# christianhbye/21cmVAE

Hardware: AMD Instinct MI355X
Metric: emulated signals/sec (batched predict) (higher is better)
Workload: dtype f16 (f32 accumulate)

## Files before the change

### 21cmvae_amd/_native.py

```python
import ctypes as C
import os
import threading
import weakref

import numpy as np

HERE = os.path.dirname(os.path.abspath(__file__))
LIB_PATH = os.environ.get("V21_LIB") or os.path.join(HERE, "libv21.so")

PREC_F32, PREC_F16, PREC_BF16 = 0, 1, 2
PRECISIONS = {"f32": PREC_F32, "fp32": PREC_F32, "float32": PREC_F32,
              "f16": PREC_F16, "fp16": PREC_F16, "float16": PREC_F16,
              "bf16": PREC_BF16, "bfloat16": PREC_BF16}
ACT_LINEAR, ACT_RELU, ACT_GAUSS = 0, 1, 2
FWD_IN_TRANSFORM, FWD_OUT_TRANSFORM, FWD_FORCE_GENERIC, FWD_NO_SMALL, FWD_FORCE_CHAIN, FWD_FORCE_JIT = 1, 2, 4, 8, 16, 32
COMM_ID_BYTES = 128


class EngineUnavailable(RuntimeError):
    """libv21.so cannot be loaded or no MI355X is visible."""


class EngineError(RuntimeError):
    """A v21_* call returned a negative status."""
# ... 40 lines not shown


class SampleOut(C.Structure):
    _fields_ = [(k, C.c_void_p) for k in SAMPLE_OUTPUTS]


_P = C.c_void_p
_F = C.POINTER(C.c_float)
SIGNATURES = {
    "v21_last_error": (C.c_char_p, []),
    "v21_version": (C.c_int, []),
    "v21_device_count": (C.c_int, [C.POINTER(C.c_int)]),
    "v21_ctx_create": (C.c_int, [C.c_int, C.POINTER(_P)]),
    "v21_ctx_destroy": (C.c_int, [_P]),
    "v21_ctx_sync": (C.c_int, [_P]),
    "v21_ctx_set_stream": (C.c_int, [_P, _P]),
    "v21_ctx_get_stream": (C.c_int, [_P, C.POINTER(_P)]),
    "v21_malloc": (C.c_int, [_P, C.c_size_t, C.POINTER(_P)]),
    "v21_free": (C.c_int, [_P, _P]),
    "v21_memcpy_h2d": (C.c_int, [_P, _P, _P, C.c_size_t]),
    "v21_memcpy_d2h": (C.c_int, [_P, _P, _P, C.c_size_t]),
    "v21_memset": (C.c_int, [_P, _P, C.c_int, C.c_size_t]),
    "v21_event_create": (C.c_int, [_P, C.POINTER(_P)]),
    "v21_event_destroy": (C.c_int, [_P, _P]),
    "v21_event_record": (C.c_int, [_P, _P]),
    "v21_event_elapsed_ms": (C.c_int, [_P, _P, _P, C.POINTER(C.c_float)]),
    "v21_mlp_create": (C.c_int, [_P, C.c_int, C.POINTER(C.c_int), C.POINTER(C.c_int), C.POINTER(_P)]),
    "v21_mlp_destroy": (C.c_int, [_P]),
    "v21_mlp_num_params": (C.c_int, [_P, C.POINTER(C.c_size_t)]),
    "v21_mlp_set_weights": (C.c_int, [_P, _F, C.c_size_t]),
    "v21_mlp_get_weights": (C.c_int, [_P, _F, C.c_size_t]),
    "v21_mlp_set_input_transform": (C.c_int, [_P, C.POINTER(AffineIn)]),
    "v21_mlp_set_output_transform": (C.c_int, [_P, C.POINTER(AffineOut)]),
    "v21_mlp_has_fused": (C.c_int, [_P, C.c_int, C.POINTER(C.c_int)]),
    "v21_mlp_jit": (C.c_int, [_P, C.c_int, C.c_int, C.POINTER(C.c_int)]),
    "v21_jit_prebuild": (C.c_int, [C.c_int, C.POINTER(C.c_int), C.POINTER(C.c_int), C.c_int, C.c_char_p]),
    "v21_mlp_forward": (C.c_int, [_P, _P, C.c_int, C.c_int64, _F, C.c_int, C.c_int]),
    "v21_mlp_forward_dev": (C.c_int, [_P, _P, C.c_int64, C.c_int64, _P, C.c_int64, C.c_int, C.c_int]),
    "v21_trainer_create": (C.c_int, [_P, C.c_int, C.c_int, C.POINTER(_P)]),
    "v21_trainer_destroy": (C.c_int, [_P]),
    "v21_trainer_set_adam": (C.c_int, [_P, C.POINTER(Adam)]),
    "v21_trainer_set_lr": (C.c_int, [_P, C.c_float]),
    "v21_trainer_get_lr": (C.c_int, [_P, C.POINTER(C.c_float)]),
    "v21_trainer_set_data": (C.c_int, [_P, C.c_int, _F, _F, _F, C.c_int64]),
    "v21_trainer_run_epoch": (C.c_int, [_P, C.POINTER(C.c_int32), C.c_int, C.POINTER(C.c_double)]),
    "v21_trainer_eval": (C.c_int, [_P, C.c_int, C.c_int, C.POINTER(C.c_double)]),
    "v21_trainer_step_dev": (C.c_int, [_P, _P, _P, _P, C.c_int, C.c_int]),
    "v21_trainer_last_step_loss": (C.c_int, [_P, C.POINTER(C.c_double)]),
    "v21_trainer_get_state": (C.c_int, [_P, C.POINTER(C.c_int64), _F, _F, C.c_size_t]),
    "v21_trainer_set_state": (C.c_int, [_P, C.c_int64, _F, _F, C.c_size_t]),
    "v21_trainer_get_grad": (C.c_int, [_P, _F, C.c_size_t]),
    "v21_trainer_use_graph": (C.c_int, [_P, C.c_int]),
    "v21_debug_poison_lds": (C.c_int, [_P, C.c_uint32]),
    "v21_debug_check_chain_jobs": (C.c_int, [_P, C.c_longlong, C.c_longlong]),
    "v21_debug_trainer_counters": (C.c_int, [_P, C.POINTER(C.c_longlong)]),
    "v21_route_forward": (C.c_int, [C.c_int, C.POINTER(C.c_int), C.POINTER(C.c_int), C.c_int, C.c_int64, C.c_int, C.c_int, C.POINTER(C.c_int)]),
    "v21_route_train": (C.c_int, [C.c_int, C.POINTER(C.c_int), C.POINTER(C.c_int), C.c_int, C.c_int, C.c_int, C.c_int, C.c_int,
                                  C.POINTER(C.c_int), C.POINTER(C.c_int)]),
    "v21_trainer_jit": (C.c_int, [_P, C.c_int, C.POINTER(C.c_int)]),
    "v21_mlp_last_route": (C.c_int, [_P, C.POINTER(C.c_int), C.POINTER(C.c_longlong)]),
    "v21_mlp_jacobian": (C.c_int, [_P, _P, C.c_int, C.c_int64, _F, _F, C.c_int, C.c_int]),
    "v21_mlp_jacobian_dev": (C.c_int, [_P, _P, C.c_int64, C.c_int64, _P, C.c_int64, _P, C.c_int, C.c_int]),
    "v21_mlp_set_likelihood": (C.c_int, [_P, _F, _F, C.c_int32]),
    "v21_mlp_loglike": (C.c_int, [_P, _P, C.c_int, C.c_int64, _F, _F, C.c_int, C.c_int]),
    "v21_mlp_loglike_dev": (C.c_int, [_P, _P, C.c_int64, C.c_int64, _P, _P, C.c_int, C.c_int]),
    "v21_route_jacobian": (C.c_int, [C.c_int, C.POINTER(C.c_int), C.POINTER(C.c_int), C.c_int, C.c_int64, C.c_int, C.POINTER(C.c_int)]),
    "v21_mlp_last_jac_route": (C.c_int, [_P, C.POINTER(C.c_int), C.POINTER(C.c_longlong)]),
    "v21_mlp_fisher": (C.c_int, [_P, _P, C.c_int, C.c_int64, _F, _F, _F, C.c_int, C.c_int]),
    "v21_mlp_fisher_dev": (C.c_int, [_P, _P, C.c_int64, C.c_int64, _P, _P, _P, C.c_int, C.c_int]),
    "v21_mlp_fit": (C.c_int, [_P, _P, C.c_int, C.c_int64, _F, C.c_int64, C.POINTER(FitOpts), _P, _F, _F, _F, C.POINTER(C.c_int32),
                              C.c_int, C.c_int]),
    "v21_mlp_fit_dev": (C.c_int, [_P, _P, C.c_int64, C.c_int64, _P, C.c_int64, C.POINTER(FitOpts), _P, _P, _P, _P, _P, C.c_int, C.c_int]),
    "v21_mlp_sample": (C.c_int, [_P, _P, C.c_int, C.c_int64, _F, C.c_int64, C.POINTER(SampleOpts), _P, C.POINTER(SampleOut),
                                 C.c_int, C.c_int]),
    "v21_mlp_sample_dev": (C.c_int, [_P, _P, C.c_int64, C.c_int64, _P, C.c_int64, C.POINTER(SampleOpts), _P, C.POINTER(SampleOut),
                                     C.c_int, C.c_int]),
    "v21_nuisance_whiten": (C.c_int, [C.POINTER(C.c_double), _F, C.c_int32, C.c_int32, C.POINTER(C.c_double), C.POINTER(C.c_double)]),
    "v21_mlp_set_nuisance": (C.c_int, [_P, C.POINTER(C.c_double), C.c_int32, C.c_int32]),
    "v21_mlp_nuisance_info": (C.c_int, [_P, C.POINTER(C.c_int32)]),
    "v21_mlp_nuisance_coef": (C.c_int, [_P, _P, C.c_int, C.c_int64, C.POINTER(C.c_double), C.c_int, C.c_int]),
    "v21_trainer_last_route": (C.c_int, [_P, C.POINTER(C.c_int), C.POINTER(C.c_int), C.POINTER(C.c_longlong), C.POINTER(C.c_longlong)]),
    "v21_route_name": (C.c_char_p, [C.c_int, C.c_int]),
    "v21_trainer_get_data_dev": (C.c_int, [_P, C.c_int, C.POINTER(_P), C.POINTER(_P), C.POINTER(_P), C.POINTER(C.c_int64)]),
    "v21_debug_clock_probe_start": (C.c_int, [_P, C.c_double, C.c_double]),
    "v21_debug_forward_clocked": (C.c_int, [_P, _P, C.c_int64, C.c_int64, _P, C.c_int64, C.c_int, C.c_int, _P]),
    "v21_debug_clock_probe_read": (C.c_int, [_P, C.POINTER(C.c_double), C.POINTER(C.c_double), C.POINTER(C.c_double), C.POINTER(C.c_int)]),
    "v21_trainer_set_vae": (C.c_int, [_P, C.c_float, C.c_int, C.c_uint64]),
    "v21_trainer_enable_stamps": (C.c_int, [_P, C.c_int]),
    "v21_trainer_chain_stamps": (C.c_int, [_P, C.POINTER(C.c_uint64), C.c_int]),
    "v21_host_alloc": (C.c_int, [_P, C.c_size_t, C.POINTER(_P)]),
    "v21_host_free": (C.c_int, [_P, _P]),
    "v21_sweep_create": (C.c_int, [C.POINTER(_P), C.c_int, C.POINTER(_P)]),
    "v21_sweep_destroy": (C.c_int, [_P]),
    "v21_sweep_run_epoch": (C.c_int, [_P, C.POINTER(C.c_int32), C.c_int, C.POINTER(C.c_double)]),
    "v21_joint_create": (C.c_int, [_P, _P, C.c_int, C.POINTER(_P)]),
    "v21_joint_destroy": (C.c_int, [_P]),
    "v21_joint_run_epoch": (C.c_int, [_P, C.POINTER(C.c_int32), C.c_int, C.POINTER(C.c_double)]),
    "v21_joint_eval": (C.c_int, [_P, C.POINTER(C.c_double)]),
    "v21_comm_get_unique_id": (C.c_int, [_P, _P]),
    "v21_comm_init": (C.c_int, [_P, C.c_int, C.c_int, _P]),
    "v21_comm_init_host": (C.c_int, [_P, C.c_int, C.c_int, C.POINTER(CommHostOps)]),
    "v21_comm_destroy": (C.c_int, [_P]),
    "v21_comm_init_null": (C.c_int, [_P, C.c_int, C.c_int]),
    "v21_comm_set_buckets": (C.c_int, [_P, C.c_int]),
    "v21_trainer_phase_timing": (C.c_int, [_P, C.c_int, C.c_int]),
    "v21_trainer_phase_times": (C.c_int, [_P, C.POINTER(C.c_double), C.POINTER(C.c_int)]),
# ... 824 lines not shown
```

### 21cmvae_amd/csrc/api_forward.hip

```cpp
#include "api_internal.h"

namespace v21 {
#define V21_DECL(a)                                                      \
  hipError_t launch_fused_##a##_F32(const FusedArgs&, hipStream_t);      \
  hipError_t launch_fused_##a##_F16x2sp(const FusedArgs&, hipStream_t);  \
  hipError_t launch_fused_##a##_BF16x2sp(const FusedArgs&, hipStream_t);
V21_ARCH_LIST(V21_DECL)
#undef V21_DECL
hipError_t launch_fused_S1_F16x2spClk(const FusedArgs&, hipStream_t);
hipError_t launch_fused_S1_BF16x2spClk(const FusedArgs&, hipStream_t);
}

typedef hipError_t (*fused_launcher)(const FusedArgs&, hipStream_t);
struct FusedEntry {
  int L;
  const int* dims;
  const int* act;
  fused_launcher fn[3];
};
#define V21_ENTRY(a) \
  {Arch##a::L, Arch##a::dims, Arch##a::act, {launch_fused_##a##_F32, launch_fused_##a##_F16x2sp, launch_fused_##a##_BF16x2sp}},
static const FusedEntry g_fused[] = {V21_ARCH_LIST(V21_ENTRY)};
#undef V21_ENTRY

// ... 329 lines not shown
  hipError_t rt = hipSuccess;
  if (route == FWD_FUSED || route == FWD_FUSED_RT) {
    CHK(ensure_stream(m, precision));
    a.x = d_x; a.ldx = ldx; a.y = d_y; a.ldy = ldy; a.n_rows = n;
    a.stream = m->d_stream[precision];
    const bool tout = (flags & V21_FWD_OUT_TRANSFORM) != 0;
    a.out_std = tout ? m->out_std : 1.0f;
    a.out_mean_scale = tout ? 1.0f : 0.0f;
    a.in_transform = (flags & V21_FWD_IN_TRANSFORM) ? 1 : 0;
    if (a.in_transform) a.tin = m->tin;
#ifdef V21_FUSED_STAMP
    a.dbg = (unsigned long long*)(getenv("V21_FUSED_DBG_PTR") ? strtoull(getenv("V21_FUSED_DBG_PTR"), nullptr, 0) : 0ull);
#endif
  }
  if (route == FWD_FUSED_RT) {
    rt = v21::jit_launch(jk, m->ctx->device, a, m->ctx->stream);
    if (rt != hipSuccess) (void)hipGetLastError();
    if (rt != hipSuccess && !force_jit) { q.jit = 0; route = decide_forward(q); }
  }
  note_route(m, route);
  if (route == FWD_TABLE) return forward_chain(m, d_x, ldx, n, d_y, ldy, precision, flags);
  if (route == FWD_GENERIC) return forward_generic(m, d_x, ldx, n, d_y, ldy, precision, flags);
  if (route == FWD_FUSED_RT) {
    if (rt == hipSuccess) return V21_OK;
    std::string why;
    v21::jit_state(jk, &why);
    return fail(V21_ERR_UNSUPPORTED, "V21_FWD_FORCE_JIT: %s (%s)", why.c_str(), hipGetErrorString(rt));
  }
  if (m->clk_stamps) {
    a.dbg = m->clk_stamps;
    HIPCHK((precision == V21_PREC_F16 ? launch_fused_S1_F16x2spClk : launch_fused_S1_BF16x2spClk)(a, m->ctx->stream));
    return V21_OK;
  }
  HIPCHK(g_fused[m->fused_id].fn[precision](a, m->ctx->stream));
  return V21_OK;
}
extern "C" int v21_mlp_forward_dev(v21_mlp* m, const float* d_x, int64_t ldx, int64_t n, float* d_y, int64_t ldy,
                                   int precision, int flags) {
  CHK(fwd_args(m, d_x && d_y, true, n, ldx, ldy, V21_DTYPE_F32, precision, flags));
  return n == 0 ? V21_OK : forward_rows(m, d_x, ldx, n, d_y, ldy, precision, flags);
}
extern "C" int v21_debug_forward_clocked(v21_mlp* m, const float* d_x, int64_t ldx, int64_t n, float* d_y, int64_t ldy, int precision,
                                         int flags, unsigned long long* d_stamps) {
  if (!m || !d_stamps) return fail(V21_ERR_ARG, "null argument");
  if (m->fused_id < 0 || g_fused[m->fused_id].dims != ArchS1::dims || (precision != V21_PREC_F16 && precision != V21_PREC_BF16))
    return fail(V21_ERR_UNSUPPORTED, "clock-stamped kernels exist for the headline stack (archs.h S1) in f16 / bf16 only");
  if (flags & (V21_FWD_FORCE_GENERIC | V21_FWD_FORCE_CHAIN | V21_FWD_FORCE_JIT)) return fail(V21_ERR_ARG, "route flags do not apply");
  m->clk_stamps = d_stamps;
  const int r = v21_mlp_forward_dev(m, d_x, ldx, n, d_y, ldy, precision, flags | V21_FWD_NO_SMALL);
  m->clk_stamps = nullptr;
  return r;
}

extern "C" int v21_mlp_jit(v21_mlp* m, int precision, int wait_ms, int* status) {
  if (!m || !status) return fail(V21_ERR_ARG, "null argument");
  if (precision < 0 || precision > 2) return fail(V21_ERR_ARG, "precision %d unknown", precision);
  *status = -1;
  if (m->fused_id >= 0) { *status = 1; return V21_OK; }
  std::string why;
  if (!v21::jit_eligible(m->L, m->dims.data(), m->act.data(), &why)) return fail(V21_ERR_UNSUPPORTED, "no fused kernel for this stack: %s", why.c_str());
  v21::JitKernel* k = jit_kernel(m, precision);
  if (!k) return fail(V21_ERR_UNSUPPORTED, "run-time compilation is switched off (V21_JIT=0) and no cached kernel exists");
  int s = v21::jit_state(k);
  if (s == v21::JIT_COMPILING && wait_ms != 0) s = v21::jit_wait(k, wait_ms);
  *status = s;
  if (s == v21::JIT_FAILED) {
    v21::jit_state(k, &why);
    return fail(V21_ERR_UNSUPPORTED, "fused kernel of this stack: %s", why.c_str());
  }
  return V21_OK;
}
extern "C" int v21_jit_prebuild(int n_layers, const int* dims, const int* act, int precision, const char* dir) {
  if (!dims || !act) return fail(V21_ERR_ARG, "null argument");
  std::string why;
  if (v21::jit_prebuild(n_layers, dims, act, precision, dir, &why) != 0) return fail(V21_ERR_UNSUPPORTED, "%s", why.c_str());
  return V21_OK;
}

extern "C" int v21_mlp_forward(v21_mlp* m, const void* x, int x_dtype, int64_t n, float* y, int precision, int flags) {
  flags &= 0xFF;
  CHK(fwd_args(m, x && y, false, n, 0, 0, x_dtype, precision, flags));
  if (n == 0) return V21_OK;
  hipStream_t st = m->ctx->stream;
  const int din = m->dims[0], dout = m->dims[m->L];
  const long long chunk = 1 << 18;
  const size_t need = (size_t)std::min<long long>(n, chunk);
  CHK(m->d_xs.reserve(need * din));
  CHK(m->d_xs64.reserve(need * din));
  CHK(m->d_ys.reserve(need * dout));
  std::vector<float> tmp;
  const bool tin = (flags & V21_FWD_IN_TRANSFORM) != 0;
  auto host_value = [&](long long r, int j) -> float {
    const v21_affine_in& a = m->tin;
    if (x_dtype == V21_DTYPE_F64) {
      const double t = ((const double*)x)[r * din + j];
      if (!tin) return (float)t;
      return par_transform_f64(t, a.log_mask[j], a.zero_floor[j], a.lo[j], a.span[j]);
    }
    const float f = ((const float*)x)[r * din + j];
    if (!tin) return f;
    return par_transform_f32(f, a.log_mask[j], a.zero_floor[j], a.lo[j], a.span[j]);
  };
  const FwdQuery hq{m->L, m->dims.data(), m->act.data(), m->fused_id >= 0, 0, precision, (long long)n, flags & ~V21_FWD_IN_TRANSFORM, (long long)dout};
  if (decide_forward(hq) == FWD_SMALL && (!tin || din <= 8)) {
    const long long ldp = p16(din);
    CHK(m->d_xpad.reserve((size_t)(n + 2) * ldp));
// ... 184 lines not shown
```

### 21cmvae_amd/csrc/fused_fwd.h

```cpp
#pragma once
#ifndef __HIPCC_RTC__
#include <hip/hip_runtime.h>
#endif

#include <type_traits>
#include <utility>

#include "../../include/v21_types.h"
#include "par_transform.h"

namespace v21 {

typedef float f32x16 __attribute__((ext_vector_type(16)));
typedef float f32x4 __attribute__((ext_vector_type(4)));
typedef _Float16 f16x8 __attribute__((ext_vector_type(8)));
typedef __bf16 bf16x8 __attribute__((ext_vector_type(8)));
typedef unsigned u32x4 __attribute__((ext_vector_type(4)));
typedef short i16x2 __attribute__((ext_vector_type(2)));
typedef float f32x2 __attribute__((ext_vector_type(2)));
typedef _Float16 f16x2 __attribute__((ext_vector_type(2)));
typedef __bf16 bf16x2 __attribute__((ext_vector_type(2)));

constexpr int kFragBytes = 1024;
constexpr int kWaves = 4;
// ... 239 lines not shown
#endif
    wait_vmcnt_barrier<N>();
#ifdef V21_FUSED_STAMP
    { unsigned long long t; asm volatile("s_memtime %0\n\ts_waitcnt lgkmcnt(0)" : "=s"(t)::"memory");
      ((unsigned long long*)(smem + G::RING * G::BLK * kFragBytes))[wave * 512 + 2 * B + 1] = t; }
#endif
    if constexpr (B >= 2 && !SPREAD) issue_block<G, B + kRing - 2>(gstream, smem, wave, lane);
  }
}

template <class G, int F> __device__ __forceinline__ const unsigned char* frag_ptr(const unsigned char* smem, int lane) {
  constexpr int B = F / G::BLK;
  return smem + ((B % G::RING) * G::BLK + (F % G::BLK)) * kFragBytes + lane * 16;
}

template <class Arch, class P>
__global__ void __launch_bounds__(64 * P::WAVES, P::WPS) fused_fwd(const FusedArgs a) {
  constexpr int kWaves = P::WAVES;
  constexpr int kBlkFrags = P::BLK, kRing = P::RING, kFusedLds = fused_lds<P>();
  (void)kFusedLds;
  extern __shared__ __attribute__((aligned(16))) unsigned char smem[];
  using G = Geo<Arch, P>;
  using frag = typename P::frag;
  using Item = typename G::Item;
  constexpr int L = G::L, CT = P::CT, EPI = P::EPI, FPI = P::FPI, IPT = G::IPT;
  constexpr int KSM = G::ks_max();
#ifndef V21_FUSED_D
#define V21_FUSED_D 2
#endif
#ifndef V21_FUSED_SPREAD
#define V21_FUSED_SPREAD 0
#endif
  constexpr int D = P::DEPTH;
  constexpr bool SPREAD = (V21_FUSED_SPREAD != 0) || spread_of<P>::value;
  constexpr int TOTAL = G::total();
  constexpr int NOUT = G::dim(L);
  constexpr int NCH = CT * 8;
  static_assert(G::act(L - 1) == 0, "output layer must be linear");
  static_assert(G::nt_of(L - 1) == 1 || G::ks_of(L - 1) > P::DEPTH, "output layer: too few k-steps per tile for the aux double buffer");
  static_assert(D <= kBlkFrags, "read-ahead must stay within one block");

  const int lane = threadIdx.x & 63;
  const int wave = __builtin_amdgcn_readfirstlane(threadIdx.x >> 6);
  const int r = lane & 31, h = lane >> 5;
  unsigned long long clk_t0 = 0, clk_r0 = 0;
  if constexpr (clk_of<P>::value) {
    asm volatile("s_memtime %0\n\ts_memrealtime %1\n\ts_waitcnt lgkmcnt(0)" : "=s"(clk_t0), "=s"(clk_r0)::"memory");
  }
  const long long wg_row0 = (long long)blockIdx.x * (kWaves * CT * 32);
  const long long row0 = wg_row0 + wave * (CT * 32);

  unsigned bufA[CT][KSM][4], bufB[CT][KSM][4];

  {
    constexpr int K0 = G::dim(0);
    static_for<CT>([&](auto ct_) __attribute__((always_inline)) {
      constexpr int ct = decltype(ct_)::value;
      const long long row = row0 + ct * 32 + r;
      const bool ok = row < a.n_rows;
      const float* xr = a.x + (ok ? row : 0) * a.ldx;
      static_for<G::ks_of(0)>([&](auto ks_) __attribute__((always_inline)) {
        constexpr int ks = decltype(ks_)::value;
        float v[EPI];
        static_for<EPI>([&](auto e_) __attribute__((always_inline)) {
          constexpr int e = decltype(e_)::value;
          constexpr int f0 = FPI * ks + 8 * (e >> 2) + (e & 3);
          constexpr int f1 = f0 + 4;
          float t = 0.f;
          if constexpr (f0 < K0) {
            const bool valid = ok && (h == 0 || f1 < K0);
            if (valid) {
              t = xr[f0 + 4 * h];
              if (a.in_transform) {
                constexpr int g1 = f1 < 8 ? f1 : 7;
                constexpr int g0 = f0 < 8 ? f0 : 7;
                const double zf = h ? a.tin.zero_floor[g1] : a.tin.zero_floor[g0];
                const int lm = h ? a.tin.log_mask[g1] : a.tin.log_mask[g0];
                const double lo = h ? a.tin.lo[g1] : a.tin.lo[g0];
                const double sp = h ? a.tin.span[g1] : a.tin.span[g0];
                t = par_transform_f32(t, lm, zf, lo, sp);
              }
            }
          }
          v[e] = t;
        });
#pragma unroll
        for (int wd = 0; wd < 4; ++wd) {
          if constexpr (EPI == 8) bufA[ct][ks][wd] = P::pack2(v[2 * wd], v[2 * wd + 1]);
          else bufA[ct][ks][wd] = __builtin_bit_cast(unsigned, v[wd]);
        }
      });
    });
  }

  static_for<kRing>([&](auto b) __attribute__((always_inline)) {
    issue_block<G, decltype(b)::value>(a.stream, smem, wave, lane);
  });

  long long wg_rows = a.n_rows - wg_row0;
  if (wg_rows > kWaves * CT * 32) wg_rows = kWaves * CT * 32;
  if (wg_rows < 0) wg_rows = 0;
  const unsigned out_bytes = (unsigned)(wg_rows * a.ldy * 4);
  __amdgpu_buffer_rsrc_t orsrc =
      __builtin_amdgcn_make_buffer_rsrc((void*)(a.y + wg_row0 * a.ldy), 0, out_bytes, 0x00020000);
  const unsigned ldy_b = (unsigned)a.ldy * 4u;
  const unsigned ovoff = (unsigned)(wave * (CT * 32) + 4 * h) * ldy_b + (unsigned)r * 4u;

  frag q[D + 1];
  f32x16 auxb[2];
  f32x16 acc[2][CT];

  auto epilogue_chunk = [&](auto g_, auto c_) __attribute__((always_inline)) {
    constexpr int GT = decltype(g_)::value;
    constexpr int c = decltype(c_)::value;
    constexpr Item t = G::tile_at(GT);
    constexpr int l = t.l, nt = t.nt;
    constexpr int ct = c / 8, pr = c % 8;
    if constexpr (l < L - 1) {
      constexpr int item = IPT * nt + (2 * pr) / EPI, e0 = (2 * pr) % EPI;
      if constexpr (item < G::ks_of(l + 1)) {
        auto& out = (l & 1) ? bufA : bufB;
        const float x0 = acc[GT & 1][ct][2 * pr], x1 = acc[GT & 1][ct][2 * pr + 1];
        if constexpr (EPI == 8) {
          unsigned w = P::pack2(x0, x1);
          if constexpr (G::act(l) != 0) {
            const i16x2 z = {0, 0};
            w = __builtin_bit_cast(unsigned, __builtin_elementwise_max(__builtin_bit_cast(i16x2, w), z));
          }
          out[ct][item][e0 / 2] = w;
        } else {
          int b0 = __builtin_bit_cast(int, x0), b1 = __builtin_bit_cast(int, x1);
          if constexpr (G::act(l) != 0) { b0 = max(b0, 0); b1 = max(b1, 0); }
          out[ct][item][e0] = (unsigned)b0;
          out[ct][item][e0 + 1] = (unsigned)b1;
        }
      }
    } else {
      const float obias = auxb[GT & 1][0], omean = auxb[GT & 1][1] * a.out_mean_scale;
      unsigned voff = ovoff + (unsigned)(32 * nt) * 4u;
      if (32 * nt + r >= NOUT) voff = 0xFFFFFFF0u;
#pragma unroll
      for (int u = 0; u < 2; ++u) {
        const int i = 2 * pr + u;
        const unsigned soff = (unsigned)(ct * 32 + (i & 3) + 8 * (i >> 2)) * ldy_b;
        float y;
        if constexpr (EPI == 8) {
          y = __builtin_fmaf(acc[GT & 1][ct][i], a.out_std, __builtin_fmaf(obias, a.out_std, omean));
        } else {
          y = (acc[GT & 1][ct][i] + obias) * a.out_std + omean;
// ... 116 lines not shown
```

### 21cmvae_amd/csrc/fused_jac.h

```cpp
#pragma once
#include "fused_fwd.h"

namespace v21 {

struct JacArgs {
  const float* x;
  long long ldx;
  const float* fac;
  float* y;
  long long ldy;
  float* jac;
  long long n_rows;
  const unsigned char* stream;
  float out_std;
  float out_mean_scale;
};

template <int IN> constexpr int jac_group() {
  static_assert(IN >= 1 && IN <= 15, "fused Jacobian: at most 15 inputs");
  return IN <= 7 ? 8 : 16;
}

template <class Arch, class P>
__global__ void __launch_bounds__(64 * P::WAVES, P::WPS) fused_jac(const JacArgs a) {
  constexpr int kWaves = P::WAVES;
  constexpr int kBlkFrags = P::BLK, kRing = P::RING;
  extern __shared__ __attribute__((aligned(16))) unsigned char smem[];
  using G = Geo<Arch, P>;
  using frag = typename P::frag;
  using Item = typename G::Item;
  constexpr int L = G::L, CT = P::CT, EPI = P::EPI, FPI = P::FPI, IPT = G::IPT;
  constexpr int KSM = G::ks_max();
  constexpr int D = P::DEPTH;
  constexpr bool SPREAD = spread_of<P>::value;
  constexpr int TOTAL = G::total();
  constexpr int K0 = G::dim(0);
  constexpr int NOUT = G::dim(L);
  constexpr int NCH = CT * 8;
  constexpr int GR = jac_group<K0>();
  constexpr int SPW = 32 * CT / GR;
  constexpr unsigned long long PAT = GR == 8 ? 0x0101010101010101ull : 0x0001000100010001ull;
  constexpr unsigned long long SPR = GR == 8 ? 0xFFull : 0xFFFFull;
  static_assert(G::act(L - 1) == 0, "output layer must be linear");
  static_assert(G::nt_of(L - 1) == 1 || G::ks_of(L - 1) > P::DEPTH, "output layer: too few k-steps per tile for the aux double buffer");
  static_assert(D <= kBlkFrags, "read-ahead must stay within one block");

  const int lane = threadIdx.x & 63;
  const int wave = __builtin_amdgcn_readfirstlane(threadIdx.x >> 6);
  const int r = lane & 31, h = lane >> 5;
  const int g_lane = r & (GR - 1);
  const bool prim_lane = g_lane == 0;
  const long long wg_vrow0 = (long long)blockIdx.x * (kWaves * CT * 32);
  const long long vrow0 = wg_vrow0 + wave * (CT * 32);
  const long long n0 = wg_vrow0 / GR;

  unsigned bufA[CT][KSM][4], bufB[CT][KSM][4];
  float fac[CT];

  static_for<CT>([&](auto ct_) __attribute__((always_inline)) {
    constexpr int ct = decltype(ct_)::value;
    const long long n = (vrow0 + ct * 32 + r) / GR;
    const bool ok = n < a.n_rows;
    const float* xr = a.x + (ok ? n : 0) * a.ldx;
    fac[ct] = (ok && g_lane >= 1 && g_lane <= K0) ? a.fac[n * K0 + g_lane - 1] : 0.f;
    static_for<G::ks_of(0)>([&](auto ks_) __attribute__((always_inline)) {
      constexpr int ks = decltype(ks_)::value;
      float v[EPI];
      static_for<EPI>([&](auto e_) __attribute__((always_inline)) {
        constexpr int e = decltype(e_)::value;
        constexpr int f0 = FPI * ks + 8 * (e >> 2) + (e & 3);
        constexpr int f1 = f0 + 4;
        float t = 0.f;
        if constexpr (f0 < K0) {
          const bool valid = ok && (h == 0 || f1 < K0);
          const int f = h ? f1 : f0;
          if (valid) t = prim_lane ? xr[f] : (f == g_lane - 1 ? 1.f : 0.f);
        }
        v[e] = t;
      });
#pragma unroll
      for (int wd = 0; wd < 4; ++wd) {
        if constexpr (EPI == 8) bufA[ct][ks][wd] = P::pack2(v[2 * wd], v[2 * wd + 1]);
        else bufA[ct][ks][wd] = __builtin_bit_cast(unsigned, v[wd]);
      }
    });
  });

  static_for<kRing>([&](auto b) __attribute__((always_inline)) {
    issue_block<G, decltype(b)::value>(a.stream, smem, wave, lane);
  });

  long long wg_sig = a.n_rows - n0;
  if (wg_sig > kWaves * CT * 32 / GR) wg_sig = kWaves * CT * 32 / GR;
  if (wg_sig < 0) wg_sig = 0;
  __amdgpu_buffer_rsrc_t yrsrc = __builtin_amdgcn_make_buffer_rsrc(
      (void*)(a.y ? a.y + n0 * a.ldy : a.jac), 0, a.y ? (unsigned)(wg_sig * a.ldy * 4) : 0u, 0x00020000);
  __amdgpu_buffer_rsrc_t jrsrc = __builtin_amdgcn_make_buffer_rsrc((void*)(a.jac + n0 * K0 * NOUT), 0, (unsigned)(wg_sig * K0 * NOUT * 4),
                                                                   0x00020000);
  const int nw0 = wave * SPW;

  frag q[D + 1];
  f32x16 auxb[2];
  f32x16 acc[2][CT];

  auto epilogue_chunk = [&](auto g_, auto c_) __attribute__((always_inline)) {
    constexpr int GT = decltype(g_)::value;
    constexpr int c = decltype(c_)::value;
    constexpr Item t = G::tile_at(GT);
    constexpr int l = t.l, nt = t.nt;
    constexpr int ct = c / 8, pr = c % 8;
    if constexpr (l < L - 1) {
      constexpr int item = IPT * nt + (2 * pr) / EPI, e0 = (2 * pr) % EPI;
      if constexpr (item < G::ks_of(l + 1)) {
        auto& out = (l & 1) ? bufA : bufB;
        float x0 = acc[GT & 1][ct][2 * pr], x1 = acc[GT & 1][ct][2 * pr + 1];
        if constexpr (G::act(l) != 0) {
          const unsigned long long m0 = (__ballot(x0 > 0.f) & PAT) * SPR;
          const unsigned long long m1 = (__ballot(x1 > 0.f) & PAT) * SPR;
          x0 = __builtin_amdgcn_inverse_ballot_w64(m0) ? x0 : 0.f;
          x1 = __builtin_amdgcn_inverse_ballot_w64(m1) ? x1 : 0.f;
        }
        if constexpr (EPI == 8) {
          out[ct][item][e0 / 2] = P::pack2(x0, x1);
        } else {
          out[ct][item][e0] = __builtin_bit_cast(unsigned, x0);
          out[ct][item][e0 + 1] = __builtin_bit_cast(unsigned, x1);
        }
      }
    } else {
      const float obias = auxb[GT & 1][0], omean = auxb[GT & 1][1] * a.out_mean_scale;
      const int bin = 32 * nt + r;
      static_for<2>([&](auto u_) __attribute__((always_inline)) {
        constexpr int i = 2 * pr + decltype(u_)::value;
        constexpr int base = ct * 32 + (i & 3) + 8 * (i >> 2);
        constexpr int gbase = base & (GR - 1);
        const int nloc = nw0 + (base - gbase) / GR;
        const int g = gbase + 4 * h;
        if constexpr (gbase == 0) {
          float yv;
          if constexpr (EPI == 8) yv = __builtin_fmaf(acc[GT & 1][ct][i], a.out_std, __builtin_fmaf(obias, a.out_std, omean));
          else yv = (acc[GT & 1][ct][i] + obias) * a.out_std + omean;
          const unsigned yoff = (h == 0 && bin < NOUT) ? ((unsigned)nloc * (unsigned)a.ldy + (unsigned)bin) * 4u : 0xFFFFFFF0u;
// ... 97 lines not shown
```

### 21cmvae_amd/csrc/par_transform.h

```cpp
#pragma once
#ifndef __HIPCC_RTC__
#include <hip/hip_runtime.h>
#endif

#include "../../include/v21_types.h"

namespace v21 {
__host__ __device__ __forceinline__ float par_transform_f32(float x, int lm, double zf, double lo, double span) {
  if (zf > 0.0 && x == 0.f) x = (float)zf;
  double t = (double)x;
  if (lm) t = (double)(float)log10(t);
  t -= lo; t /= span; t *= 2.0; t -= 1.0;
  return (float)t;
}
__host__ __device__ __forceinline__ float par_transform_f64(double t, int lm, double zf, double lo, double span) {
  if (zf > 0.0 && t == 0.0) t = zf;
  if (lm) t = log10(t);
  t -= lo; t /= span; t *= 2.0; t -= 1.0;
  return (float)t;
}
}
```

### include/v21.h

```cpp
#ifndef V21_H
#define V21_H

#include <stddef.h>
#include <stdint.h>

#ifdef __cplusplus
extern "C" {
#endif

typedef struct v21_ctx v21_ctx;
typedef struct v21_mlp v21_mlp;
typedef struct v21_trainer v21_trainer;

enum {
  V21_OK = 0,
  V21_ERR_ARG = -1,
  V21_ERR_HIP = -2,
  V21_ERR_UNSUPPORTED = -3,
  V21_ERR_STATE = -4,
  V21_ERR_COMM = -5
};

enum { V21_PREC_F32 = 0, V21_PREC_F16 = 1, V21_PREC_BF16 = 2 };
enum { V21_ACT_LINEAR = 0, V21_ACT_RELU = 1, V21_ACT_GAUSS = 2 };
// ... 61 lines not shown
int v21_mlp_loglike(v21_mlp* mlp, const void* x, int x_dtype, int64_t n, float* lnl, float* grad, int precision, int flags);
int v21_mlp_loglike_dev(v21_mlp* mlp, const float* d_x, int64_t ldx, int64_t n, float* d_lnl, float* d_grad, int precision,
                        int flags);
int v21_route_jacobian(int n_layers, const int* dims, const int* act, int precision, int64_t n, int flags, int* route);
int v21_mlp_last_jac_route(v21_mlp* mlp, int* route, long long counts[4]);

int v21_mlp_fisher(v21_mlp* mlp, const void* x, int x_dtype, int64_t n, float* fisher, float* lnl, float* grad, int precision, int flags);
int v21_mlp_fisher_dev(v21_mlp* mlp, const float* d_x, int64_t ldx, int64_t n, float* d_fisher, float* d_lnl, float* d_grad,
                       int precision, int flags);
int v21_mlp_fit(v21_mlp* mlp, const void* x0, int x_dtype, int64_t n, const float* data, int64_t n_data, const v21_fit_opts* opts,
                void* x_hat, float* lnl, float* lnl_start, float* fisher, int32_t* status, int precision, int flags);
int v21_mlp_fit_dev(v21_mlp* mlp, const float* d_x0, int64_t ldx, int64_t n, const float* d_data, int64_t n_data,
                    const v21_fit_opts* opts, float* d_x_hat, float* d_lnl, float* d_lnl_start, float* d_fisher, int32_t* d_status,
                    int precision, int flags);

int v21_mlp_sample(v21_mlp* mlp, const void* x0, int x_dtype, int64_t n, const float* data, int64_t n_data, const v21_sample_opts* opts,
                   const double* eps_start, const v21_sample_out* out, int precision, int flags);
int v21_mlp_sample_dev(v21_mlp* mlp, const float* d_x0, int64_t ldx, int64_t n, const float* d_data, int64_t n_data,
                       const v21_sample_opts* opts, const double* d_eps_start, const v21_sample_out* out, int precision, int flags);

int v21_nuisance_whiten(const double* basis, const float* inv_var, int32_t n_modes, int32_t out_dim, double* q, double* r);
int v21_mlp_set_nuisance(v21_mlp* mlp, const double* basis, int32_t n_modes, int32_t out_dim);
int v21_mlp_nuisance_info(v21_mlp* mlp, int32_t* n_modes);
int v21_mlp_nuisance_coef(v21_mlp* mlp, const void* x, int x_dtype, int64_t n, double* coef, int precision, int flags);

typedef struct {
  float lr, beta1, beta2, eps;
} v21_adam;

int v21_trainer_create(v21_mlp* mlp, int precision, int max_batch, v21_trainer** out);
int v21_trainer_destroy(v21_trainer* tr);
int v21_trainer_set_adam(v21_trainer* tr, const v21_adam* cfg);
int v21_trainer_set_lr(v21_trainer* tr, float lr);
int v21_trainer_get_lr(v21_trainer* tr, float* lr);
int v21_trainer_set_data(v21_trainer* tr, int which , const float* x,
                         const float* y, const float* row_weight, int64_t n);
int v21_trainer_run_epoch(v21_trainer* tr, const int32_t* perm, int batch, double* loss);
int v21_trainer_eval(v21_trainer* tr, int which, int batch, double* loss);
int v21_trainer_get_data_dev(v21_trainer* tr, int which, const float** x, const float** y, const float** row_weight, int64_t* n);
int v21_trainer_step_dev(v21_trainer* tr, const float* d_x, const float* d_y,
                         const float* d_row_weight, int n_rows, int global_rows);
int v21_trainer_last_step_loss(v21_trainer* tr, double* loss);
int v21_trainer_get_state(v21_trainer* tr, int64_t* iter, float* m, float* v, size_t n);
int v21_trainer_set_state(v21_trainer* tr, int64_t iter, const float* m, const float* v,
                          size_t n);
int v21_trainer_get_grad(v21_trainer* tr, float* g, size_t n);
typedef struct v21_joint v21_joint;
int v21_joint_create(v21_trainer* ae, v21_trainer* em, int latent_layer, v21_joint** out);
int v21_joint_destroy(v21_joint* j);
int v21_joint_run_epoch(v21_joint* j, const int32_t* perm , int batch, double* losses );
int v21_joint_eval(v21_joint* j, double* losses );
int v21_trainer_use_graph(v21_trainer* tr, int enable);
int v21_debug_poison_lds(v21_ctx* ctx, uint32_t pattern);
int v21_debug_clock_probe_start(v21_ctx* ctx, double duration_ms, double period_us);
int v21_debug_forward_clocked(v21_mlp* mlp, const float* d_x, int64_t ldx, int64_t n, float* d_y, int64_t ldy, int precision,
                              int flags, unsigned long long* d_stamps);
int v21_debug_clock_probe_read(v21_ctx* ctx, double* ghz_mean, double* ghz_min, double* ghz_max, int* samples);
int v21_debug_check_chain_jobs(v21_trainer* tr, long long fw_bytes, long long bw_bytes);
int v21_route_forward(int n_layers, const int* dims, const int* act, int precision, int64_t n, int flags, int rt_ready, int* route);
int v21_route_train(int n_layers, const int* dims, const int* act, int precision, int max_batch, int rows, int nranks, int rt_ready, int* fwd, int* upd);
int v21_mlp_last_route(v21_mlp* mlp, int* route, long long counts[8]);
int v21_trainer_last_route(v21_trainer* tr, int* fwd, int* upd, long long fwd_counts[8], long long upd_counts[8]);
const char* v21_route_name(int kind, int route);
int v21_trainer_phase_timing(v21_trainer* tr, int steps, int cut);
int v21_trainer_phase_times(v21_trainer* tr, double* ms, int* steps);
int v21_debug_trainer_counters(v21_trainer* tr, long long out[4]);
int v21_trainer_enable_stamps(v21_trainer* tr, int enable);
int v21_trainer_chain_stamps(v21_trainer* tr, uint64_t* out, int n);
int v21_trainer_set_vae(v21_trainer* tr, float kl_weight, int sample, uint64_t seed);

typedef struct v21_sweep v21_sweep;
int v21_sweep_create(v21_trainer** trainers, int count, v21_sweep** out);
int v21_sweep_destroy(v21_sweep* sw);
int v21_sweep_run_epoch(v21_sweep* sw, const int32_t* perm, int batch, double* losses);

#define V21_COMM_ID_BYTES 128
typedef struct v21_comm_host_ops {
  void* user;
  int (*allreduce_sum_f32)(void* user, float* buf, size_t n);
  int (*reduce_scatter_sum_f32)(void* user, float* buf, size_t n_per);
  int (*allgather_f32)(void* user, float* buf, size_t n_per);
} v21_comm_host_ops;
int v21_comm_get_unique_id(v21_ctx* ctx, void* id );
int v21_comm_init(v21_ctx* ctx, int nranks, int rank, const void* id);
int v21_comm_init_host(v21_ctx* ctx, int nranks, int rank, const v21_comm_host_ops* ops);
int v21_comm_init_null(v21_ctx* ctx, int nranks, int rank);
int v21_comm_set_buckets(v21_ctx* ctx, int buckets);
int v21_comm_destroy(v21_ctx* ctx);
int v21_comm_set_sharded(v21_ctx* ctx, int on);
int v21_comm_info(v21_ctx* ctx, int* nranks, int* rank, int* transport);
int v21_comm_allreduce_f32(v21_ctx* ctx, float* d_buf, size_t n);
int v21_comm_reduce_scatter_f32(v21_ctx* ctx, float* d_buf, size_t n_per);
int v21_comm_allgather_f32(v21_ctx* ctx, float* d_buf, size_t n_per);

#ifdef __cplusplus
}
#endif
#endif
```

Before: 1.194 billion.

## Overlap input loads with weight prefetch and use fast log10 in transform

The fused forward and jacobian kernels now load raw input rows into registers first, pin them with empty asm barriers, and issue the weight-ring prefetch before applying the parameter transform and packing. This lets the global input loads overlap with the weight stream issue. The log10 in the input transform is replaced by a double-precision polynomial that falls back to the library log10 when float rounding is ambiguous, which keeps results bit-identical. It also adds a host debug entry point that compares the fast and reference transforms, and it costs extra registers to hold the inputs.

```diff
diff --git a/21cmvae_amd/_native.py b/21cmvae_amd/_native.py
--- a/21cmvae_amd/_native.py
+++ b/21cmvae_amd/_native.py
@@ -116,6 +116,7 @@
     "v21_trainer_get_grad": (C.c_int, [_P, _F, C.c_size_t]),
     "v21_trainer_use_graph": (C.c_int, [_P, C.c_int]),
     "v21_debug_poison_lds": (C.c_int, [_P, C.c_uint32]),
+    "v21_debug_par_transform_host": (C.c_int, [C.POINTER(AffineIn), C.c_int, _P, C.c_int64, _P, _P]),
     "v21_debug_check_chain_jobs": (C.c_int, [_P, C.c_longlong, C.c_longlong]),
     "v21_debug_trainer_counters": (C.c_int, [_P, C.POINTER(C.c_longlong)]),
     "v21_route_forward": (C.c_int, [C.c_int, C.POINTER(C.c_int), C.POINTER(C.c_int), C.c_int, C.c_int64, C.c_int, C.c_int, C.POINTER(C.c_int)]),
diff --git a/21cmvae_amd/csrc/api_forward.hip b/21cmvae_amd/csrc/api_forward.hip
--- a/21cmvae_amd/csrc/api_forward.hip
+++ b/21cmvae_amd/csrc/api_forward.hip
@@ -405,6 +405,16 @@
   return r;
 }
 
+extern "C" int v21_debug_par_transform_host(const v21_affine_in* t, int col, const float* x, int64_t n, float* out_fast, float* out_ref) {
+  if (!t || !x || !out_fast || !out_ref) return fail(V21_ERR_ARG, "null argument");
+  if (col < 0 || col >= 8 || n < 0) return fail(V21_ERR_ARG, "column %d of 8, %lld values", col, (long long)n);
+  for (int64_t i = 0; i < n; ++i) {
+    out_fast[i] = par_transform_f32(x[i], t->log_mask[col], t->zero_floor[col], t->lo[col], t->span[col]);
+    out_ref[i] = par_transform_f32_ref(x[i], t->log_mask[col], t->zero_floor[col], t->lo[col], t->span[col]);
+  }
+  return V21_OK;
+}
+
 extern "C" int v21_mlp_jit(v21_mlp* m, int precision, int wait_ms, int* status) {
   if (!m || !status) return fail(V21_ERR_ARG, "null argument");
   if (precision < 0 || precision > 2) return fail(V21_ERR_ARG, "precision %d unknown", precision);
diff --git a/21cmvae_amd/csrc/fused_fwd.h b/21cmvae_amd/csrc/fused_fwd.h
--- a/21cmvae_amd/csrc/fused_fwd.h
+++ b/21cmvae_amd/csrc/fused_fwd.h
@@ -315,49 +315,70 @@
 
   unsigned bufA[CT][KSM][4], bufB[CT][KSM][4];
 
-  {
-    constexpr int K0 = G::dim(0);
-    static_for<CT>([&](auto ct_) __attribute__((always_inline)) {
-      constexpr int ct = decltype(ct_)::value;
-      const long long row = row0 + ct * 32 + r;
-      const bool ok = row < a.n_rows;
-      const float* xr = a.x + (ok ? row : 0) * a.ldx;
-      static_for<G::ks_of(0)>([&](auto ks_) __attribute__((always_inline)) {
-        constexpr int ks = decltype(ks_)::value;
-        float v[EPI];
-        static_for<EPI>([&](auto e_) __attribute__((always_inline)) {
-          constexpr int e = decltype(e_)::value;
-          constexpr int f0 = FPI * ks + 8 * (e >> 2) + (e & 3);
-          constexpr int f1 = f0 + 4;
-          float t = 0.f;
-          if constexpr (f0 < K0) {
-            const bool valid = ok && (h == 0 || f1 < K0);
-            if (valid) {
-              t = xr[f0 + 4 * h];
-              if (a.in_transform) {
-                constexpr int g1 = f1 < 8 ? f1 : 7;
-                constexpr int g0 = f0 < 8 ? f0 : 7;
-                const double zf = h ? a.tin.zero_floor[g1] : a.tin.zero_floor[g0];
-                const int lm = h ? a.tin.log_mask[g1] : a.tin.log_mask[g0];
-                const double lo = h ? a.tin.lo[g1] : a.tin.lo[g0];
-                const double sp = h ? a.tin.span[g1] : a.tin.span[g0];
-                t = par_transform_f32(t, lm, zf, lo, sp);
-              }
-            }
-          }
-          v[e] = t;
-        });
-#pragma unroll
-        for (int wd = 0; wd < 4; ++wd) {
-          if constexpr (EPI == 8) bufA[ct][ks][wd] = P::pack2(v[2 * wd], v[2 * wd + 1]);
-          else bufA[ct][ks][wd] = __builtin_bit_cast(unsigned, v[wd]);
-        }
+  constexpr int K0 = G::dim(0);
+  constexpr int KS0 = G::ks_of(0);
+  float xv[CT][KS0][EPI];
+  static_for<CT>([&](auto ct_) __attribute__((always_inline)) {
+    constexpr int ct = decltype(ct_)::value;
+    const long long row = row0 + ct * 32 + r;
+    const bool ok = row < a.n_rows;
+    const float* xr = a.x + (ok ? row : 0) * a.ldx;
+    static_for<KS0>([&](auto ks_) __attribute__((always_inline)) {
+      constexpr int ks = decltype(ks_)::value;
+      static_for<EPI>([&](auto e_) __attribute__((always_inline)) {
+        constexpr int e = decltype(e_)::value;
+        constexpr int f0 = FPI * ks + 8 * (e >> 2) + (e & 3);
+        constexpr int f1 = f0 + 4;
+        float t = 0.f;
+        if constexpr (f0 < K0) {
+          if (ok && (h == 0 || f1 < K0)) t = xr[f0 + 4 * h];
+        }
+        xv[ct][ks][e] = t;
       });
     });
-  }
+  });
+  static_for<CT * KS0 * EPI>([&](auto i_) __attribute__((always_inline)) {
+    constexpr int i = decltype(i_)::value, ks = i / EPI % KS0, e = i % EPI;
+    if constexpr (FPI * ks + 8 * (e >> 2) + (e & 3) < K0) {
+      float& p = xv[i / (KS0 * EPI)][ks][e];
+      asm volatile("" : "+v"(p)::"memory");
+    }
+  });
 
   static_for<kRing>([&](auto b) __attribute__((always_inline)) {
     issue_block<G, decltype(b)::value>(a.stream, smem, wave, lane);
+  });
+
+  static_for<CT>([&](auto ct_) __attribute__((always_inline)) {
+    constexpr int ct = decltype(ct_)::value;
+    const bool ok = row0 + ct * 32 + r < a.n_rows;
+    static_for<KS0>([&](auto ks_) __attribute__((always_inline)) {
+      constexpr int ks = decltype(ks_)::value;
+      float v[EPI];
+      static_for<EPI>([&](auto e_) __attribute__((always_inline)) {
+        constexpr int e = decltype(e_)::value;
+        constexpr int f0 = FPI * ks + 8 * (e >> 2) + (e & 3);
+        constexpr int f1 = f0 + 4;
+        float t = xv[ct][ks][e];
+        if constexpr (f0 < K0) {
+          if (a.in_transform && ok && (h == 0 || f1 < K0)) {
+            constexpr int g1 = f1 < 8 ? f1 : 7;
+            constexpr int g0 = f0 < 8 ? f0 : 7;
+            const double zf = h ? a.tin.zero_floor[g1] : a.tin.zero_floor[g0];
+            const int lm = h ? a.tin.log_mask[g1] : a.tin.log_mask[g0];
+            const double lo = h ? a.tin.lo[g1] : a.tin.lo[g0];
+            const double sp = h ? a.tin.span[g1] : a.tin.span[g0];
+            t = par_transform_f32(t, lm, zf, lo, sp);
+          }
+        }
+        v[e] = t;
+      });
+#pragma unroll
+      for (int wd = 0; wd < 4; ++wd) {
+        if constexpr (EPI == 8) bufA[ct][ks][wd] = P::pack2(v[2 * wd], v[2 * wd + 1]);
+        else bufA[ct][ks][wd] = __builtin_bit_cast(unsigned, v[wd]);
+      }
+    });
   });
 
   long long wg_rows = a.n_rows - wg_row0;
diff --git a/21cmvae_amd/csrc/fused_jac.h b/21cmvae_amd/csrc/fused_jac.h
--- a/21cmvae_amd/csrc/fused_jac.h
+++ b/21cmvae_amd/csrc/fused_jac.h
@@ -57,24 +57,59 @@
   unsigned bufA[CT][KSM][4], bufB[CT][KSM][4];
   float fac[CT];
 
+  constexpr int KS0 = G::ks_of(0);
+  float xv[CT][KS0][EPI];
   static_for<CT>([&](auto ct_) __attribute__((always_inline)) {
     constexpr int ct = decltype(ct_)::value;
     const long long n = (vrow0 + ct * 32 + r) / GR;
     const bool ok = n < a.n_rows;
     const float* xr = a.x + (ok ? n : 0) * a.ldx;
     fac[ct] = (ok && g_lane >= 1 && g_lane <= K0) ? a.fac[n * K0 + g_lane - 1] : 0.f;
-    static_for<G::ks_of(0)>([&](auto ks_) __attribute__((always_inline)) {
+    static_for<KS0>([&](auto ks_) __attribute__((always_inline)) {
+      constexpr int ks = decltype(ks_)::value;
+      static_for<EPI>([&](auto e_) __attribute__((always_inline)) {
+        constexpr int e = decltype(e_)::value;
+        constexpr int f0 = FPI * ks + 8 * (e >> 2) + (e & 3);
+        constexpr int f1 = f0 + 4;
+        float t = 0.f;
+        if constexpr (f0 < K0) {
+          if (ok && prim_lane && (h == 0 || f1 < K0)) t = xr[h ? f1 : f0];
+        }
+        xv[ct][ks][e] = t;
+      });
+    });
+  });
+  static_for<CT * KS0 * EPI>([&](auto i_) __attribute__((always_inline)) {
+    constexpr int i = decltype(i_)::value, ks = i / EPI % KS0, e = i % EPI;
+    if constexpr (FPI * ks + 8 * (e >> 2) + (e & 3) < K0) {
+      float& p = xv[i / (KS0 * EPI)][ks][e];
+      asm volatile("" : "+v"(p)::"memory");
+    }
+  });
+  static_for<CT>([&](auto ct_) __attribute__((always_inline)) {
+    float& p = fac[decltype(ct_)::value];
+    asm volatile("" : "+v"(p)::"memory");
+  });
+
+  static_for<kRing>([&](auto b) __attribute__((always_inline)) {
+    issue_block<G, decltype(b)::value>(a.stream, smem, wave, lane);
+  });
+
+  static_for<CT>([&](auto ct_) __attribute__((always_inline)) {
+    constexpr int ct = decltype(ct_)::value;
+    const bool ok = (vrow0 + ct * 32 + r) / GR < a.n_rows;
+    static_for<KS0>([&](auto ks_) __attribute__((always_inline)) {
       constexpr int ks = decltype(ks_)::value;
       float v[EPI];
       static_for<EPI>([&](auto e_) __attribute__((always_inline)) {
         constexpr int e = decltype(e_)::value;
         constexpr int f0 = FPI * ks + 8 * (e >> 2) + (e & 3);
         constexpr int f1 = f0 + 4;
-        float t = 0.f;
+        float t = xv[ct][ks][e];
         if constexpr (f0 < K0) {
           const bool valid = ok && (h == 0 || f1 < K0);
           const int f = h ? f1 : f0;
-          if (valid) t = prim_lane ? xr[f] : (f == g_lane - 1 ? 1.f : 0.f);
+          if (valid && !prim_lane) t = f == g_lane - 1 ? 1.f : 0.f;
         }
         v[e] = t;
       });
@@ -84,10 +119,6 @@
         else bufA[ct][ks][wd] = __builtin_bit_cast(unsigned, v[wd]);
       }
     });
-  });
-
-  static_for<kRing>([&](auto b) __attribute__((always_inline)) {
-    issue_block<G, decltype(b)::value>(a.stream, smem, wave, lane);
   });
 
   long long wg_sig = a.n_rows - n0;
diff --git a/21cmvae_amd/csrc/par_transform.h b/21cmvae_amd/csrc/par_transform.h
--- a/21cmvae_amd/csrc/par_transform.h
+++ b/21cmvae_amd/csrc/par_transform.h
@@ -6,10 +6,47 @@
 #include "../../include/v21_types.h"
 
 namespace v21 {
+constexpr double kLogEps = 0x1p-45;
+
+__host__ __device__ __forceinline__ bool log10f_fast(float x, float* out) {
+  const long long b = __builtin_bit_cast(long long, (double)x);
+  int e = (int)(b >> 52) - 1023;
+  double m = __builtin_bit_cast(double, (b & 0x000FFFFFFFFFFFFFll) | 0x3FF0000000000000ll);
+  if (m > 1.4142135623730951) { m *= 0.5; e += 1; }
+  const double s = (m - 1.0) / (m + 1.0);
+  const double z = s * s;
+  double p = 1.0 / 19.0;
+  p = __builtin_fma(p, z, 1.0 / 17.0);
+  p = __builtin_fma(p, z, 1.0 / 15.0);
+  p = __builtin_fma(p, z, 1.0 / 13.0);
+  p = __builtin_fma(p, z, 1.0 / 11.0);
+  p = __builtin_fma(p, z, 1.0 / 9.0);
+  p = __builtin_fma(p, z, 1.0 / 7.0);
+  p = __builtin_fma(p, z, 1.0 / 5.0);
+  p = __builtin_fma(p, z, 1.0 / 3.0);
+  p = __builtin_fma(p, z, 1.0);
+  const double lm = (s * 0.86858896380650365530) * p;
+  const double l = __builtin_fma((double)e, 0.30102999566398119521, lm);
+  const float a = (float)__builtin_fma(l, -kLogEps, l), c = (float)__builtin_fma(l, kLogEps, l);
+  *out = a;
+  return a == c;
+}
+
+__host__ __device__ __forceinline__ float par_transform_f32_ref(float x, int lm, double zf, double lo, double span) {
+  if (zf > 0.0 && x == 0.f) x = (float)zf;
+  double t = (double)x;
+  if (lm) t = (double)(float)log10(t);
+  t -= lo; t /= span; t *= 2.0; t -= 1.0;
+  return (float)t;
+}
 __host__ __device__ __forceinline__ float par_transform_f32(float x, int lm, double zf, double lo, double span) {
   if (zf > 0.0 && x == 0.f) x = (float)zf;
   double t = (double)x;
-  if (lm) t = (double)(float)log10(t);
+  if (lm) {
+    float l;
+    if (x > 0.f && x <= 3.40282346638528859812e38f && log10f_fast(x, &l)) t = (double)l;
+    else t = (double)(float)log10(t);
+  }
   t -= lo; t /= span; t *= 2.0; t -= 1.0;
   return (float)t;
 }
diff --git a/include/v21.h b/include/v21.h
--- a/include/v21.h
+++ b/include/v21.h
@@ -137,6 +137,7 @@
 int v21_joint_eval(v21_joint* j, double* losses );
 int v21_trainer_use_graph(v21_trainer* tr, int enable);
 int v21_debug_poison_lds(v21_ctx* ctx, uint32_t pattern);
+int v21_debug_par_transform_host(const v21_affine_in* t, int col, const float* x, int64_t n, float* out_fast, float* out_ref);
 int v21_debug_clock_probe_start(v21_ctx* ctx, double duration_ms, double period_us);
 int v21_debug_forward_clocked(v21_mlp* mlp, const float* d_x, int64_t ldx, int64_t n, float* d_y, int64_t ldy, int precision,
                               int flags, unsigned long long* d_stamps);
```

After: 1.192 billion (median of 3 runs). About the same (-0.2%).
